# bluenote-1577/skani

Measured on NVIDIA H100. Metric: genome-pairs/sec, skani triangle 5k x 5 Mbp synthetic, higher is better.
Workload: dtype u64

## Files before the change

### skani_b200/csrc/seeding.cu

```cuda
#include <cub/cub.cuh>
#include <thrust/iterator/transform_iterator.h>

#include <algorithm>
#include <cstdlib>
#include <cstring>

#include "sk_core.cuh"
#include "sk_internal.h"

namespace sk {

uint64_t count_launch(sk_ctx* ctx, uint64_t n) {
  ctx->launches += n;
  return ctx->launches;
}

constexpr int PACK_THREADS = 256;
constexpr uint32_t UCOARSE_SHIFT = 8;

__device__ __forceinline__ uint32_t find_contig(const uint32_t* __restrict__ cuoff, uint32_t u, uint32_t lo_hint, uint32_t hi_hint) {
  uint32_t lo = lo_hint, hi = hi_hint;
  while (hi - lo > 1) {
    uint32_t mid = (lo + hi) >> 1;
    if (cuoff[mid] <= u) lo = mid; else hi = mid;
  }
  return lo;
}
__device__ __forceinline__ uint32_t contig_of_unit(const uint32_t* __restrict__ ucoarse, const uint32_t* __restrict__ cuoff, uint32_t u) {
  const uint32_t lo = __ldg(ucoarse + (u >> UCOARSE_SHIFT)), hi = __ldg(ucoarse + (u >> UCOARSE_SHIFT) + 1) + 1;
  return find_contig(cuoff, u, lo, hi);
}

__global__ void __launch_bounds__(PACK_THREADS)
pack_kernel(const uint8_t* __restrict__ ascii, const uint64_t* __restrict__ coff, const uint32_t* __restrict__ cuoff,
            const uint32_t* __restrict__ clen, const uint32_t* __restrict__ ucoarse, uint32_t u_begin, uint32_t n_units,
            uint64_t* __restrict__ P, uint32_t* __restrict__ NM, int small_n) {
  const uint32_t u = u_begin + blockIdx.x * PACK_THREADS + threadIdx.x;
  if (u >= n_units) return;
  const uint32_t ci = contig_of_unit(ucoarse, cuoff, u);
  const uint32_t ul = u - cuoff[ci];
  const uint32_t len = clen[ci];
  const uint32_t nvalid = min(32u, len - 32u * ul);
  const uint8_t* src = ascii + coff[ci] + 32ull * ul;
  const uintptr_t addr = (uintptr_t)src;
  const uint32_t* wp = (const uint32_t*)(addr & ~(uintptr_t)3);
  const uint32_t sh = (uint32_t)(addr & 3) * 8;
  const uint32_t nwords = (nvalid + (uint32_t)(addr & 3) + 3) >> 2;
  uint32_t w[9];
#pragma unroll
  for (int i = 0; i < 9; i++) w[i] = (i < (int)nwords) ? __ldg(wp + i) : 0u;
  uint64_t packed = 0;
  uint32_t nm = 0;
#pragma unroll
  for (int i = 0; i < 8; i++) {
    const uint32_t r = __funnelshift_r(w[i], w[i + 1], sh);
    uint32_t c8, n4;
    pack_word(r, c8, n4, small_n != 0);
    packed |= (uint64_t)c8 << (8 * i);
    nm |= n4 << (4 * i);
  }
  if (nvalid < 32u) { packed &= (1ull << (2 * nvalid)) - 1ull; nm &= (1u << nvalid) - 1u; }
  P[u] = packed;
  NM[u] = nm;
}

constexpr int HASH_THREADS = 128;

template <int V>
__device__ __forceinline__ uint64_t xorshift_var(uint64_t key, uint32_t s, uint32_t c) {
  const uint32_t lo = (uint32_t)key, hi = (uint32_t)(key >> 32);
  uint32_t hs, ls;
  asm("mul.hi.u32 %0, %1, %2;" : "=r"(hs) : "r"(hi), "r"(c));
  if (V == 1) ls = __funnelshift_r(lo, hi, s);
  else { uint32_t t; asm("mul.hi.u32 %0, %1, %2;" : "=r"(t) : "r"(lo), "r"(c)); ls = t + hi * c; }
  return ((uint64_t)(hi ^ hs) << 32) | (uint64_t)(lo ^ ls);
}
template <int V>
__device__ __forceinline__ uint32_t unit_pass_mask_var(uint64_t lo, uint64_t hi, uint32_t nm_lo, uint32_t nm_hi, uint32_t n, uint32_t ul,
                                                       uint32_t seed_mask32, uint64_t threshold, uint32_t c24, uint32_t c14, uint32_t c28) {
  const uint32_t valid = unit_valid_mask(n, ul);
  if (valid == 0) return 0;
  const uint64_t clo = ~lo, chi = ~hi;
  const uint64_t tlo = pair_reverse64(hi), thi = pair_reverse64(lo);
  const uint32_t c[4] = {(uint32_t)clo, (uint32_t)(clo >> 32), (uint32_t)chi, (uint32_t)(chi >> 32)};
  const uint32_t t[4] = {(uint32_t)tlo, (uint32_t)(tlo >> 32), (uint32_t)thi, (uint32_t)(thi >> 32)};
  uint32_t pass = 0;
#pragma unroll
  for (uint32_t j = 0; j < 32; j++) {
    const uint32_t orv = 24 + 2 * j, ofw = 62 - 2 * j;
    const uint32_t rs = funnel_r32(c[orv >> 5], c[(orv >> 5) + 1], orv & 31) & seed_mask32;
    const uint32_t fs = funnel_r32(t[ofw >> 5], t[(ofw >> 5) + 1], ofw & 31) & seed_mask32;
    const uint32_t seed = fs < rs ? fs : rs;
    uint64_t key = ~((uint64_t)seed * 0x200001ull);
    key = xorshift_var<V>(key, 24, c24);
    key = key * 265ull;
    key = xorshift_var<V>(key, 14, c14);
    key = key * 21ull;
    key = xorshift_var<V>(key, 28, c28);
    key = key * 0x80000001ull;
    if (key < threshold) pass |= 1u << j;
  }
  pass &= valid;
  if ((nm_lo | nm_hi) != 0 && pass != 0) pass &= ~unit_n_suppress_mask(n, ul, nm_lo, nm_hi, pass);
  return pass;
}

template <int V>
__global__ void __launch_bounds__(HASH_THREADS)
hashpass_kernel(const uint64_t* __restrict__ P, const uint32_t* __restrict__ NM, const uint32_t* __restrict__ ucoarse,
                const uint32_t* __restrict__ cuoff, const uint32_t* __restrict__ clen, uint32_t n_units,
                uint64_t seed_mask, uint64_t threshold, uint32_t* __restrict__ PM, uint32_t c24, uint32_t c14, uint32_t c28,
                uint32_t scalar_k) {
  uint32_t u = blockIdx.x * HASH_THREADS + threadIdx.x;
  if (u >= n_units) return;
  const uint64_t hi = P[u];
  const uint64_t lo_raw = u ? P[u - 1] : 0ull;
  const uint32_t nhi = NM[u];
  const uint32_t nlo_raw = u ? NM[u - 1] : 0u;
  const uint32_t ci = contig_of_unit(ucoarse, cuoff, u);
  const uint32_t ul = u - cuoff[ci];
  const uint32_t n = clen[ci];
  const uint64_t lo = ul ? lo_raw : 0ull;
  const uint32_t nlo = ul ? nlo_raw : 0u;
  if (V == 0) PM[u] = unit_pass_mask_fast(lo, hi, nlo, nhi, n, ul, (uint32_t)seed_mask, threshold, scalar_k);
  else PM[u] = unit_pass_mask_var<V>(lo, hi, nlo, nhi, n, ul, (uint32_t)seed_mask, threshold, c24, c14, c28);
}

__global__ void __launch_bounds__(256)
expand_kernel(const uint64_t* __restrict__ P, const uint32_t* __restrict__ ucoarse, const uint32_t* __restrict__ cuoff,
              const uint32_t* __restrict__ clocal, uint32_t n_units, const uint32_t* __restrict__ PM,
              const uint32_t* __restrict__ uoff, uint64_t seed_mask, uint64_t threshold_marker,
              uint32_t* __restrict__ pv_kmer, uint32_t* __restrict__ pv_pos, uint32_t* __restrict__ pv_cc,
              uint64_t* __restrict__ mkv) {
  uint32_t u = blockIdx.x * 256 + threadIdx.x;
  if (u >= n_units) return;
  uint32_t pass = PM[u];
  if (pass == 0) return;
  uint32_t ci = contig_of_unit(ucoarse, cuoff, u);
  uint32_t ul = u - cuoff[ci];
  uint64_t hi = P[u];
  uint64_t lo = ul ? P[u - 1] : 0ull;
  WindowCtx w = make_window_ctx(lo, hi);
  uint32_t o = uoff[u];
  uint32_t cl = clocal[ci];
  while (pass) {
    uint32_t j = __ffs(pass) - 1;
    pass &= pass - 1;
    bool canon;
    uint32_t seed = window_seed(w, j, seed_mask, &canon);
    pv_kmer[o] = seed;
    pv_pos[o] = 32u * ul + j;
    pv_cc[o] = (cl << 1) | (canon ? 1u : 0u);
    mkv[o] = (mm_hash64(seed) < threshold_marker) ? window_marker(w, j) : ~0ull;
    o++;
  }
}

__global__ void gather_u32_kernel(const uint32_t* __restrict__ src, const uint32_t* __restrict__ idx, uint32_t n,
                                  uint32_t src_len, uint32_t total, uint32_t* __restrict__ dst) {
  uint32_t i = blockIdx.x * blockDim.x + threadIdx.x;
  if (i >= n) return;
  uint32_t k = idx[i];
  dst[i] = (k >= src_len) ? total : src[k];
}

__global__ void gather_u32_tail_kernel(const uint32_t* __restrict__ src, const uint32_t* __restrict__ idx, uint32_t n,
                                       uint32_t src_len, const uint32_t* __restrict__ tail, int tail_is_mask,
                                       uint32_t* __restrict__ dst) {
  uint32_t i = blockIdx.x * blockDim.x + threadIdx.x;
  if (i >= n) return;
  uint32_t k = idx[i];
  if (k >= src_len) { const uint32_t t = tail[src_len - 1]; dst[i] = src[src_len - 1] + (tail_is_mask ? (uint32_t)__popc(t) : t); }
  else dst[i] = src[k];
}

__global__ void marker_flag_kernel(const uint64_t* __restrict__ mkv, uint32_t n, uint32_t* __restrict__ flag) {
  uint32_t i = blockIdx.x * blockDim.x + threadIdx.x;
  if (i < n) flag[i] = (mkv[i] != ~0ull) ? 1u : 0u;
}
__global__ void marker_scatter_kernel(const uint64_t* __restrict__ mkv, const uint32_t* __restrict__ scan, uint32_t n,
                                      uint64_t* __restrict__ out) {
  uint32_t i = blockIdx.x * blockDim.x + threadIdx.x;
  if (i < n && mkv[i] != ~0ull) out[scan[i]] = mkv[i];
}

__global__ void iota_local_kernel(const uint64_t* __restrict__ seg_off, uint32_t* __restrict__ vals) {
  uint32_t g = blockIdx.x;
  uint64_t b = seg_off[g], e = seg_off[g + 1];
  for (uint64_t i = b + (uint64_t)blockIdx.y * blockDim.x + threadIdx.x; i < e; i += (uint64_t)blockDim.x * gridDim.y) vals[i] = (uint32_t)(i - b);
}

__global__ void kview_keys_kernel(const uint64_t* __restrict__ seg_off, const uint32_t* __restrict__ pv_kmer, uint32_t kbits,
                                  uint32_t ibits, uint64_t* __restrict__ keys, uint32_t* __restrict__ vals) {
  const uint32_t g = blockIdx.x;
  const uint64_t b = seg_off[g], e = seg_off[g + 1];
  for (uint64_t i = b + (uint64_t)blockIdx.y * blockDim.x + threadIdx.x; i < e; i += (uint64_t)blockDim.x * gridDim.y) {
    const uint64_t k = ((uint64_t)g << kbits) | pv_kmer[i];
    if (ibits) keys[i] = (k << ibits) | (uint64_t)(i - b);
    else { keys[i] = k; vals[i] = (uint32_t)(i - b); }
  }
}
__global__ void marker_keys_kernel(const uint64_t* __restrict__ seg_off, uint64_t* __restrict__ mk) {
  const uint32_t g = blockIdx.x;
  const uint64_t b = seg_off[g], e = seg_off[g + 1];
  for (uint64_t i = b + (uint64_t)blockIdx.y * blockDim.x + threadIdx.x; i < e; i += (uint64_t)blockDim.x * gridDim.y) mk[i] |= (uint64_t)g << (2 * MARKER_K);
}


__global__ void kview_gather_kernel(const uint64_t* __restrict__ seg_off, const uint64_t* __restrict__ skmer,
                                    const uint32_t* __restrict__ perm, const uint32_t* __restrict__ pv_pos,
                                    const uint32_t* __restrict__ pv_cc, uint32_t* __restrict__ kv_pos,
                                    uint32_t* __restrict__ kv_cc, uint32_t* __restrict__ head, uint32_t ibits, uint32_t gshift,
                                    uint32_t n) {
  const uint32_t i = blockIdx.x * blockDim.x + threadIdx.x;
  if (i >= n) return;
  const uint64_t imask = (1ull << ibits) - 1;
  const uint64_t k = skmer[i];
  const uint64_t b = seg_off[k >> gshift];
  const uint32_t r = ibits ? (uint32_t)(k & imask) : perm[i];
  kv_pos[i] = pv_pos[b + r];
  kv_cc[i] = pv_cc[b + r];
  head[i] = (i == 0 || (k >> ibits) != (skmer[i - 1] >> ibits)) ? 1u : 0u;
}

__global__ void groups_kernel(const uint64_t* __restrict__ seg_off, const uint64_t* __restrict__ skmer, uint64_t kmask,
                              const uint32_t* __restrict__ head, const uint32_t* __restrict__ hscan,
                              uint32_t n_genomes, uint32_t* __restrict__ ukmer, uint32_t* __restrict__ ustart, uint32_t ibits,
                              uint32_t gshift, uint32_t n) {
  const uint32_t i = blockIdx.x * blockDim.x + threadIdx.x;
  if (i < n && head[i]) {
    const uint64_t k = skmer[i];
    const uint32_t g = (uint32_t)(k >> gshift);
    const uint32_t gid = hscan[i];
    ukmer[gid] = (uint32_t)((k >> ibits) & kmask);
    ustart[gid + g] = (uint32_t)(i - seg_off[g]);
  }
  if (i < n_genomes) {
    const uint32_t g = i;
    const uint64_t b = seg_off[g], e = seg_off[g + 1];
    const uint32_t next_gid = (e < n) ? hscan[e] : hscan[n - 1] + head[n - 1];
    ustart[next_gid + g] = (uint32_t)(e - b);
  }
}

__global__ void mult_kernel(const uint64_t* __restrict__ seg_off, const uint32_t* __restrict__ head,
                            const uint32_t* __restrict__ hscan, const uint32_t* __restrict__ perm,
                            const uint32_t* __restrict__ ustart, uint16_t* __restrict__ pv_mult,
                            const uint64_t* __restrict__ skmer, uint32_t ibits, uint32_t gshift, uint32_t n) {
  const uint32_t i = blockIdx.x * blockDim.x + threadIdx.x;
  if (i >= n) return;
  const uint64_t imask = (1ull << ibits) - 1;
  const uint64_t k = skmer[i];
  const uint32_t g = (uint32_t)(k >> gshift);
  const uint32_t gid = hscan[i] + head[i] - 1;
  const uint32_t cntv = ustart[gid + g + 1] - ustart[gid + g];
  const uint32_t r = ibits ? (uint32_t)(k & imask) : perm[i];
  pv_mult[seg_off[g] + r] = (uint16_t)min(cntv, 65535u);
}

__global__ void bucket_kernel(const uint64_t* __restrict__ uk_off, const uint32_t* __restrict__ ukmer, uint32_t shift,
                              uint32_t* __restrict__ ubucket) {
  const uint32_t g = blockIdx.x;
  const uint32_t* uk = ukmer + uk_off[g];
  const uint32_t n = (uint32_t)(uk_off[g + 1] - uk_off[g]);
  for (uint32_t b = threadIdx.x; b <= UBUCKETS; b += blockDim.x) {
    uint32_t lo = 0, hi = n;
    while (lo < hi) {
      uint32_t mid = (lo + hi) >> 1;
      if ((uk[mid] >> shift) < b) lo = mid + 1; else hi = mid;
    }
    ubucket[(size_t)g * (UBUCKETS + 1) + b] = lo;
  }
}

__global__ void marker_head_kernel(const uint64_t* __restrict__ seg_off, const uint64_t* __restrict__ mk,
                                   uint32_t* __restrict__ head) {
  uint32_t g = blockIdx.x;
  uint64_t b = seg_off[g], e = seg_off[g + 1];
  for (uint64_t i = b + (uint64_t)blockIdx.y * blockDim.x + threadIdx.x; i < e; i += (uint64_t)blockDim.x * gridDim.y) head[i] = (i == b || mk[i] != mk[i - 1]) ? 1u : 0u;
}
__global__ void marker_compact_kernel(const uint64_t* __restrict__ mk, const uint32_t* __restrict__ head,
                                      const uint32_t* __restrict__ hscan, uint32_t n, uint64_t mask, uint64_t* __restrict__ out) {
  uint32_t i = blockIdx.x * blockDim.x + threadIdx.x;
  if (i < n && head[i]) out[hscan[i]] = mk[i] & mask;
}
__global__ void gather_scan_at_kernel(const uint32_t* __restrict__ scan, const uint64_t* __restrict__ at, uint32_t n,
                                      uint64_t len, uint32_t total, uint64_t* __restrict__ out) {
  uint32_t i = blockIdx.x * blockDim.x + threadIdx.x;
  if (i < n) out[i] = (at[i] >= len) ? (uint64_t)total : (uint64_t)scan[at[i]];
}

__global__ void gather_scan_at_tail_kernel(const uint32_t* __restrict__ scan, const uint64_t* __restrict__ at, uint32_t n,
                                           uint64_t len, const uint32_t* __restrict__ flag, uint64_t* __restrict__ out) {
  uint32_t i = blockIdx.x * blockDim.x + threadIdx.x;
  if (i < n) out[i] = (at[i] >= len) ? (uint64_t)(scan[len - 1] + flag[len - 1]) : (uint64_t)scan[at[i]];
}

static void* mbox_alloc(sk_ctx* ctx, size_t bytes) {
  bytes = (bytes + 63) & ~(size_t)63;
  for (;;) {
    if (ctx->mbox_block < ctx->mbox_blocks.size()) {
      auto& b = ctx->mbox_blocks[ctx->mbox_block];
      if (ctx->mbox_pos + bytes <= b.second) { void* p = b.first + ctx->mbox_pos; ctx->mbox_pos += bytes; return p; }
      ctx->mbox_block++; ctx->mbox_pos = 0;
      continue;
    }
    uint8_t* p = nullptr;
// ... 156 lines not shown
    DTmp<uint32_t> vals, perm, head, hscan;
    DTmp<uint64_t> keys, skmer;
    SK_CUDA(keys.alloc(S, ctx)); SK_CUDA(skmer.alloc(S, ctx));
    SK_CUDA(head.alloc(S + 1, ctx)); SK_CUDA(hscan.alloc(S + 1, ctx));
    const uint32_t kbits = std::min(32u, 2 * set->sp.k);
    const uint32_t gbits = G > 1 ? 32 - (uint32_t)__builtin_clz(G - 1) : 0;
    const uint64_t kmask = (kbits >= 64) ? ~0ull : ((1ull << kbits) - 1);
    uint64_t max_rec = 1;
    for (uint32_t g = 0; g < G; g++) max_rec = std::max<uint64_t>(max_rec, set->seed_off[g + 1] - set->seed_off[g]);
    uint32_t ibits = max_rec > 1 ? 64 - (uint32_t)__builtin_clzll(max_rec - 1) : 1;
    if (ibits + kbits + gbits > 64 || getenv("SK_KVIEW_SORT_PAIRS")) ibits = 0;
    if (!ibits) { SK_CUDA(vals.alloc(S, ctx)); SK_CUDA(perm.alloc(S, ctx)); }
    kview_keys_kernel<<<dim3(G, 8), 256, 0, st>>>(d_seed_off.p, set->pv_kmer, kbits, ibits, keys.p, vals.p); count_launch(ctx);
    size_t tb = 0;
    DTmp<uint8_t> tmp;
    if (ibits) {
      SK_CUDA(cub::DeviceRadixSort::SortKeys(nullptr, tb, keys.p, skmer.p, (int)S, (int)ibits, (int)(ibits + kbits + gbits), st));
      SK_CUDA(tmp.alloc(tb, ctx));
      SK_CUDA(cub::DeviceRadixSort::SortKeys(tmp.p, tb, keys.p, skmer.p, (int)S, (int)ibits, (int)(ibits + kbits + gbits), st));
    } else {
      SK_CUDA(cub::DeviceRadixSort::SortPairs(nullptr, tb, keys.p, skmer.p, vals.p, perm.p, (int)S, 0, (int)(kbits + gbits), st));
      SK_CUDA(tmp.alloc(tb, ctx));
      SK_CUDA(cub::DeviceRadixSort::SortPairs(tmp.p, tb, keys.p, skmer.p, vals.p, perm.p, (int)S, 0, (int)(kbits + gbits), st));
    }
    count_launch(ctx);
    const uint32_t gshift = ibits + kbits;
    kview_gather_kernel<<<div_up(S, 256), 256, 0, st>>>(d_seed_off.p, skmer.p, perm.p, set->pv_pos, set->pv_cc, set->kv_pos,
                                                        set->kv_cc, head.p, ibits, gshift, (uint32_t)S); count_launch(ctx);
    SK_TRY(scan_exclusive<uint32_t>(ctx, head.p, hscan.p, S));
    DTmp<uint64_t> d_ukoff;
    SK_CUDA(d_ukoff.alloc(G + 1, ctx));
    gather_scan_at_tail_kernel<<<div_up(G + 1, 256), 256, 0, st>>>(hscan.p, d_seed_off.p, G + 1, S, head.p, d_ukoff.p); count_launch(ctx);
    SK_CUDA(cudaMemcpyAsync(h_ukoff, d_ukoff.p, (size_t)(G + 1) * 8, cudaMemcpyDeviceToHost, st));
    SK_CUDA(ctx->arena.alloc((void**)&set->ukmer, S * 4));
    SK_CUDA(ctx->arena.alloc((void**)&set->ustart, (size_t)(S + G + 1) * 4));
    groups_kernel<<<div_up(std::max<uint64_t>(S, G), 256), 256, 0, st>>>(d_seed_off.p, skmer.p, kmask, head.p, hscan.p, G, set->ukmer,
                                                                         set->ustart, ibits, gshift, (uint32_t)S); count_launch(ctx);
    mult_kernel<<<div_up(S, 256), 256, 0, st>>>(d_seed_off.p, head.p, hscan.p, perm.p, set->ustart, set->pv_mult, skmer.p, ibits, gshift,
                                                (uint32_t)S); count_launch(ctx);
  } else {
    set->U = 0;
    SK_CUDA(ctx->arena.alloc((void**)&set->ukmer, 4));
    SK_CUDA(ctx->arena.alloc((void**)&set->ustart, (size_t)(G + 1) * 4));
    SK_CUDA(cudaMemsetAsync(set->ustart, 0, (size_t)(G + 1) * 4, st));
    for (uint32_t g = 0; g <= G; g++) h_ukoff[g] = 0;
  }
  SK_CUDA(cudaStreamSynchronize(st));
  for (uint32_t g = 0; g <= G; g++) set->uk_off[g] = h_ukoff[g];
  set->U = (size_t)set->uk_off[G];
  const size_t MR = raw_mk_off[G];
  set->mk_off.assign(G + 1, 0);
  if (MR > 0) {
    if (MR >= (1ull << 31)) { ctx->err = "sub-batch has >= 2^31 markers"; return SK_ERR_PARAM; }
    SK_CUDA(d_rawmk_off.alloc(G + 1, ctx));
    SK_CUDA(h2d_small(ctx, d_rawmk_off.p, raw_mk_off, (G + 1) * 8));
    DTmp<uint64_t> sorted;
    SK_CUDA(sorted.alloc(MR, ctx));
    size_t tb = 0;
    const uint32_t mgbits = G > 1 ? 32 - (uint32_t)__builtin_clz(G - 1) : 0;
    const bool global_sort = 2 * MARKER_K + mgbits <= 64;
    DTmp<uint8_t> tmp;
    if (global_sort) {
      marker_keys_kernel<<<dim3(G, 8), 256, 0, st>>>(d_rawmk_off.p, d_marker_raw); count_launch(ctx);
      SK_CUDA(cub::DeviceRadixSort::SortKeys(nullptr, tb, d_marker_raw, sorted.p, (int)MR, 0, (int)(2 * MARKER_K + mgbits), st));
      SK_CUDA(tmp.alloc(tb, ctx));
      SK_CUDA(cub::DeviceRadixSort::SortKeys(tmp.p, tb, d_marker_raw, sorted.p, (int)MR, 0, (int)(2 * MARKER_K + mgbits), st));
    } else {
      SK_CUDA(cub::DeviceSegmentedRadixSort::SortKeys(nullptr, tb, d_marker_raw, sorted.p, (int)MR, (int)G, d_rawmk_off.p,
                                                      d_rawmk_off.p + 1, 0, 2 * MARKER_K, st));
      SK_CUDA(tmp.alloc(tb, ctx));
      SK_CUDA(cub::DeviceSegmentedRadixSort::SortKeys(tmp.p, tb, d_marker_raw, sorted.p, (int)MR, (int)G, d_rawmk_off.p,
                                                      d_rawmk_off.p + 1, 0, 2 * MARKER_K, st));
    }
    count_launch(ctx);
    DTmp<uint32_t> head, hscan;
    SK_CUDA(head.alloc(MR, ctx)); SK_CUDA(hscan.alloc(MR, ctx));
    marker_head_kernel<<<dim3(G, 8), 256, 0, st>>>(d_rawmk_off.p, sorted.p, head.p); count_launch(ctx);
    SK_TRY(scan_exclusive<uint32_t>(ctx, head.p, hscan.p, MR));
    SK_CUDA(ctx->arena.alloc((void**)&set->markers, MR * 8));
    marker_compact_kernel<<<div_up(MR, 256), 256, 0, st>>>(sorted.p, head.p, hscan.p, (uint32_t)MR, global_sort ? ((1ull << (2 * MARKER_K)) - 1) : ~0ull, set->markers); count_launch(ctx);
    DTmp<uint64_t> d_mkoff;
    SK_CUDA(d_mkoff.alloc(G + 1, ctx));
    gather_scan_at_tail_kernel<<<div_up(G + 1, 256), 256, 0, st>>>(hscan.p, d_rawmk_off.p, G + 1, MR, head.p, d_mkoff.p); count_launch(ctx);
    SK_CUDA(cudaMemcpyAsync(h_mkoff, d_mkoff.p, (size_t)(G + 1) * 8, cudaMemcpyDeviceToHost, st));
    SK_CUDA(cudaStreamSynchronize(st));
    for (uint32_t g = 0; g <= G; g++) set->mk_off[g] = h_mkoff[g];
    set->M = (size_t)set->mk_off[G];
  } else {
    set->M = 0;
    SK_CUDA(ctx->arena.alloc((void**)&set->markers, 8));
  }
  return SK_OK;
}

struct PopcOp { using result_type = uint32_t; __device__ __forceinline__ uint32_t operator()(uint32_t m) const { return (uint32_t)__popc(m); } };

int sketch_batch_device(sk_ctx* ctx, const SeedSrc& src, const uint64_t* contig_off, uint32_t n_contigs,
                        const uint32_t* genome_of_contig, uint32_t n_genomes, const sk_sketch_params* sp, sk_sketch_set** out) {
  cudaStream_t st = ctx->stream;
  const uint32_t G = n_genomes;
  sk_sketch_set* set = new sk_sketch_set();
  set->ctx = ctx; set->sp = *sp; set->G = G;
  struct Guard { sk_sketch_set* s; ~Guard() { if (s) { free_set_device(s); delete s; } } } guard{set};

  std::vector<uint64_t> coff(n_contigs + 1);
  std::vector<uint32_t> cuoff(n_contigs + 1), clen(n_contigs), clocal(n_contigs);
  set->ctg_off.assign(G + 1, 0);
  set->total_len.assign(G, 0);
  set->ctg_len.resize(n_contigs);
  uint64_t units = 0;
  uint32_t prev_g = 0, rank = 0;
  for (uint32_t i = 0; i < n_contigs; i++) {
    uint64_t len = contig_off[i + 1] - contig_off[i];
    if (contig_off[i + 1] < contig_off[i] || len >= (1ull << 32) - 65536) { ctx->err = "contig length out of range (u32 positions, src/types.rs:52; pos + 20000 must not wrap, src/chain.rs:743)"; return SK_ERR_PARAM; }
    uint32_t g = genome_of_contig[i];
    if (g >= G || g < prev_g) { ctx->err = "genome_of_contig must be non-decreasing and < n_genomes"; return SK_ERR_PARAM; }
    if (g != prev_g || i == 0) rank = 0;
    prev_g = g;
    if (rank >= (1u << 30)) { ctx->err = "contig index exceeds 30 bits (src/types.rs:136)"; return SK_ERR_PARAM; }
    coff[i] = contig_off[i] - src.ascii_base;
    cuoff[i] = (uint32_t)units;
    clen[i] = (uint32_t)len;
    clocal[i] = rank++;
    set->ctg_len[i] = (uint32_t)len;
    set->ctg_off[g + 1]++;
    set->total_len[g] += len;
    units += (len + 31) / 32;
    if (units >= (1ull << 31)) { ctx->err = "sub-batch too large (>= 2^31 units)"; return SK_ERR_PARAM; }
  }
  coff[n_contigs] = contig_off[n_contigs] - src.ascii_base;
  cuoff[n_contigs] = (uint32_t)units;
  for (uint32_t g = 0; g < G; g++) set->ctg_off[g + 1] += set->ctg_off[g];
  set->C = n_contigs;
  set->name_rank.resize(G);
  for (uint32_t g = 0; g < G; g++) set->name_rank[g] = g;
  const uint32_t NU = (uint32_t)units;
  const uint32_t n_packed = std::min(src.n_packed, n_contigs);
  if (n_packed && (!src.d_P || !src.d_NM)) { ctx->err = "packed contigs without unit arrays"; return SK_ERR_PARAM; }
  std::vector<uint32_t> ucoarse(((size_t)NU >> UCOARSE_SHIFT) + 2, n_contigs ? n_contigs - 1 : 0);
  {
    uint32_t ci = 0;
    for (size_t j = 0; ((uint64_t)j << UCOARSE_SHIFT) < NU; j++) {
      const uint32_t u = (uint32_t)(j << UCOARSE_SHIFT);
      while (ci + 1 < n_contigs && cuoff[ci + 1] <= u) ci++;
      ucoarse[j] = ci;
    }
  }

  SK_CUDA(ctx->arena.alloc((void**)&set->d_ctg_len, std::max<size_t>(n_contigs, 1) * 4));
  SK_CUDA(ctx->arena.alloc((void**)&set->ctg_rec_off, (size_t)(n_contigs + G + 1) * 4));
  set->seed_off.assign(G + 1, 0);

  DTmp<uint64_t> d_coff, Pown;
  DTmp<uint32_t> d_cuoff, d_clen, d_clocal, d_ucoarse, NMown, PM, uoff;
  mbox_reset(ctx);
  uint64_t* h_raw_mk_off = (uint64_t*)mbox_alloc(ctx, (size_t)(G + 1) * 8);
  if (h_raw_mk_off) for (uint32_t g = 0; g <= G; g++) h_raw_mk_off[g] = 0;
  DTmp<uint64_t> mkv, mraw;
  if (NU > 0) {
    SK_CUDA(d_coff.alloc(n_contigs + 1, ctx)); SK_CUDA(d_cuoff.alloc(n_contigs + 1, ctx));
    SK_CUDA(d_clen.alloc(n_contigs, ctx)); SK_CUDA(d_clocal.alloc(n_contigs, ctx)); SK_CUDA(d_ucoarse.alloc(ucoarse.size(), ctx));
    SK_CUDA(h2d_small(ctx, d_coff.p, coff.data(), (n_contigs + 1) * 8));
    SK_CUDA(h2d_small(ctx, d_cuoff.p, cuoff.data(), (n_contigs + 1) * 4));
    SK_CUDA(h2d_small(ctx, d_clen.p, clen.data(), n_contigs * 4));
    SK_CUDA(h2d_small(ctx, d_clocal.p, clocal.data(), n_contigs * 4));
    SK_CUDA(h2d_small(ctx, d_ucoarse.p, ucoarse.data(), ucoarse.size() * 4));
    SK_CUDA(h2d_small(ctx, set->d_ctg_len, clen.data(), n_contigs * 4));
    uint64_t* P = src.d_P; uint32_t* NM = src.d_NM;
    if (!P) { SK_CUDA(Pown.alloc(NU, ctx)); SK_CUDA(NMown.alloc(NU, ctx)); P = Pown.p; NM = NMown.p; }
    SK_CUDA(PM.alloc(NU, ctx)); SK_CUDA(uoff.alloc(NU, ctx));

    const uint32_t u_ascii = cuoff[n_packed];
    if (u_ascii < NU) {
      if (!src.d_ascii) { ctx->err = "ASCII contigs without a device buffer"; return SK_ERR_PARAM; }
      SK_LAUNCH(ctx, "pack_kernel", (pack_kernel<<<div_up(NU - u_ascii, PACK_THREADS), PACK_THREADS, 0, st>>>(
          src.d_ascii, d_coff.p, d_cuoff.p, d_clen.p, d_ucoarse.p, u_ascii, NU, P, NM, ctx->seed_scalar ? 1 : 0)));
    }
    const uint64_t seed_mask = ~0ull >> (64 - 2 * sp->k);
    const uint64_t thr = ~0ull / sp->c, thr_m = ~0ull / sp->marker_c;
    {
      const uint32_t scalar_k = ctx->seed_scalar ? sp->k : 0;
      const int hv = (getenv("SK_HASHPASS_VARIANT") && !scalar_k) ? atoi(getenv("SK_HASHPASS_VARIANT")) : 0;
      const uint32_t c24 = 1u << 8, c14 = 1u << 18, c28 = 1u << 4;
      const uint32_t grid = div_up(NU, HASH_THREADS);
      if (hv == 1) SK_LAUNCH(ctx, "hashpass_kernel", (hashpass_kernel<1><<<grid, HASH_THREADS, 0, st>>>(P, NM, d_ucoarse.p, d_cuoff.p, d_clen.p, NU, seed_mask, thr, PM.p, c24, c14, c28, scalar_k)));
      else if (hv == 2) SK_LAUNCH(ctx, "hashpass_kernel", (hashpass_kernel<2><<<grid, HASH_THREADS, 0, st>>>(P, NM, d_ucoarse.p, d_cuoff.p, d_clen.p, NU, seed_mask, thr, PM.p, c24, c14, c28, scalar_k)));
      else SK_LAUNCH(ctx, "hashpass_kernel", (hashpass_kernel<0><<<grid, HASH_THREADS, 0, st>>>(P, NM, d_ucoarse.p, d_cuoff.p, d_clen.p, NU, seed_mask, thr, PM.p, c24, c14, c28, scalar_k)));
    }
    {
      auto cnt_it = thrust::make_transform_iterator((const uint32_t*)PM.p, PopcOp());
      size_t tb = 0;
      SK_CUDA(cub::DeviceScan::ExclusiveSum(nullptr, tb, cnt_it, uoff.p, (int)NU, st));
      DTmp<uint8_t> tmp;
      SK_CUDA(tmp.alloc(tb, ctx));
      SK_CUDA(cub::DeviceScan::ExclusiveSum(tmp.p, tb, cnt_it, uoff.p, (int)NU, st));
      count_launch(ctx, 2);
    }
    DTmp<uint32_t> d_crec;
    SK_CUDA(d_crec.alloc(n_contigs + 1, ctx));
    gather_u32_tail_kernel<<<div_up(n_contigs + 1, 256), 256, 0, st>>>(uoff.p, d_cuoff.p, n_contigs + 1, NU, PM.p, 1, d_crec.p); count_launch(ctx);
    uint32_t* crec = (uint32_t*)mbox_alloc(ctx, (size_t)(n_contigs + 1) * 4);
    if (!crec || !h_raw_mk_off) { ctx->err = "out of pinned host memory"; return SK_ERR_NOMEM; }
    SK_CUDA(cudaMemcpyAsync(crec, d_crec.p, (size_t)(n_contigs + 1) * 4, cudaMemcpyDeviceToHost, st));
    SK_CUDA(cudaStreamSynchronize(st));
    const uint32_t S = crec[n_contigs];
    set->S = S;
    SK_CUDA(ctx->arena.alloc((void**)&set->pv_kmer, std::max<size_t>(S, 1) * 4));
    SK_CUDA(ctx->arena.alloc((void**)&set->pv_pos, std::max<size_t>(S, 1) * 4));
    SK_CUDA(ctx->arena.alloc((void**)&set->pv_cc, std::max<size_t>(S, 1) * 4));
    SK_CUDA(mkv.alloc(S, ctx));
    SK_LAUNCH(ctx, "expand_kernel", (expand_kernel<<<div_up(NU, 256), 256, 0, st>>>(
        P, d_ucoarse.p, d_cuoff.p, d_clocal.p, NU, PM.p, uoff.p, seed_mask, thr_m, set->pv_kmer, set->pv_pos, set->pv_cc, mkv.p)));
    std::vector<uint32_t> crl(n_contigs + G + 1, 0);
    for (uint32_t g = 0; g < G; g++) {
      uint64_t c0 = set->ctg_off[g], c1 = set->ctg_off[g + 1];
      uint32_t base = (c0 < n_contigs) ? crec[c0] : S;
      set->seed_off[g] = base;
      for (uint64_t c = c0; c < c1; c++) crl[c + g] = crec[c] - base;
      uint32_t endrec = (c1 < n_contigs) ? crec[c1] : S;
      crl[c1 + g] = endrec - base;
    }
    set->seed_off[G] = S;
    SK_CUDA(h2d_small(ctx, set->ctg_rec_off, crl.data(), (size_t)(n_contigs + G) * 4));
    if (S > 0) {
      DTmp<uint32_t> mflag, mscan;
      SK_CUDA(mflag.alloc(S, ctx)); SK_CUDA(mscan.alloc(S, ctx));
      marker_flag_kernel<<<div_up(S, 256), 256, 0, st>>>(mkv.p, S, mflag.p); count_launch(ctx);
      SK_TRY(scan_exclusive<uint32_t>(ctx, mflag.p, mscan.p, S));
      DTmp<uint64_t> d_so, d_mo;
      SK_CUDA(d_so.alloc(G + 1, ctx)); SK_CUDA(d_mo.alloc(G + 1, ctx));
      SK_CUDA(h2d_small(ctx, d_so.p, set->seed_off.data(), (G + 1) * 8));
      SK_CUDA(mraw.alloc(S, ctx));
      marker_scatter_kernel<<<div_up(S, 256), 256, 0, st>>>(mkv.p, mscan.p, S, mraw.p); count_launch(ctx);
      gather_scan_at_tail_kernel<<<div_up(G + 1, 256), 256, 0, st>>>(mscan.p, d_so.p, G + 1, S, mflag.p, d_mo.p); count_launch(ctx);
      SK_CUDA(cudaMemcpyAsync(h_raw_mk_off, d_mo.p, (size_t)(G + 1) * 8, cudaMemcpyDeviceToHost, st));
    }
  } else {
    set->S = 0;
    SK_CUDA(ctx->arena.alloc((void**)&set->pv_kmer, 4)); SK_CUDA(ctx->arena.alloc((void**)&set->pv_pos, 4)); SK_CUDA(ctx->arena.alloc((void**)&set->pv_cc, 4));
    SK_CUDA(cudaMemsetAsync(set->ctg_rec_off, 0, (size_t)(n_contigs + G + 1) * 4, st));
  }
  Pown.release(); NMown.release(); PM.release(); uoff.release(); mkv.release();
  if (!h_raw_mk_off) { ctx->err = "out of pinned host memory"; return SK_ERR_NOMEM; }
  SK_TRY(build_views(ctx, set, mraw.p, h_raw_mk_off));
  SK_CUDA(cudaStreamSynchronize(st));
  guard.s = nullptr;
  *out = set;
  return SK_OK;
}

}
```

### skani_b200/csrc/sk_core.cuh

```cuda
#pragma once
#include <stdint.h>

#if defined(__CUDACC__)
#define SK_HD __host__ __device__ __forceinline__
#else
#define SK_HD inline
#endif

namespace sk {

constexpr int MARKER_K = 21;
constexpr uint32_t UNIT_BASES = 32;

SK_HD uint64_t mm_hash64(uint64_t key) {
  key = ~(key + (key << 21));
  key = key ^ (key >> 24);
  key = key * 265;
  key = key ^ (key >> 14);
  key = key * 21;
  key = key ^ (key >> 28);
  key = key + (key << 31);
  return key;
}

// ... 56 lines not shown
  w.t_lo = pair_reverse64(hi); w.t_hi = pair_reverse64(lo);
  return w;
}
SK_HD uint64_t window_f21(const WindowCtx& w, uint32_t j) { return extract128(w.t_lo, w.t_hi, 62 - 2 * j) & ((1ull << 42) - 1); }
SK_HD uint64_t window_r21(const WindowCtx& w, uint32_t j) { return extract128(w.c_lo, w.c_hi, 24 + 2 * j) & ((1ull << 42) - 1); }

SK_HD uint32_t window_seed(const WindowCtx& w, uint32_t j, uint64_t seed_mask, bool* canonical) {
  uint64_t fs = window_f21(w, j) & seed_mask;
  uint64_t rs = window_r21(w, j) & seed_mask;
  *canonical = fs < rs;
  return (uint32_t)(fs < rs ? fs : rs);
}
SK_HD uint64_t window_marker(const WindowCtx& w, uint32_t j) {
  uint64_t f = window_f21(w, j), r = window_r21(w, j);
  return r > f ? f : r;
}

SK_HD uint32_t unit_valid_mask(uint32_t n, uint32_t ul) {
  if (n < 2 * MARKER_K) return 0;
  uint32_t q = (n - 20) / 4;
  uint64_t e_lo = 20, e_hi = 4ull * q + 20;
  uint64_t b = 32ull * ul;
  uint32_t m = 0xFFFFFFFFu;
  if (b + 32 <= e_lo || b >= e_hi) return 0;
  if (b < e_lo) m &= 0xFFFFFFFFu << (uint32_t)(e_lo - b);
  if (b + 32 > e_hi) m &= 0xFFFFFFFFu >> (uint32_t)(b + 32 - e_hi);
  return m;
}

SK_HD uint32_t unit_n_suppress_mask(uint32_t n, uint32_t ul, uint32_t nm_lo, uint32_t nm_hi, uint32_t cand) {
  uint64_t nm = ((uint64_t)nm_hi << 32) | nm_lo;
  if (nm == 0 || cand == 0) return 0;
  uint32_t q = (n - 20) / 4;
  uint32_t sup = 0;
  for (uint32_t j = 0; j < 32; j++) {
    if (!((cand >> j) & 1u)) continue;
    int64_t e = 32ll * ul + j;
    int64_t lane = (e - 20) / (int64_t)q;
    int64_t lb = e - 20;
    int64_t lane_lb = lane * (int64_t)q + 20;
    if (lane_lb > lb) lb = lane_lb;
    int64_t base0 = 32ll * ((int64_t)ul - 1);
    uint32_t r_lo = (uint32_t)(lb - base0), r_hi = (uint32_t)(e - base0);
    uint64_t span = (r_hi - r_lo == 63) ? ~0ull : (((1ull << (r_hi - r_lo + 1)) - 1) << r_lo);
    if (nm & span) sup |= 1u << j;
  }
  return sup;
}

SK_HD uint32_t unit_valid_mask_scalar(uint32_t n, uint32_t ul) {
  if (n < 2 * MARKER_K) return 0;
  const uint64_t e_lo = 20, e_hi = n;
  const uint64_t b = 32ull * ul;
  uint32_t m = 0xFFFFFFFFu;
  if (b + 32 <= e_lo || b >= e_hi) return 0;
  if (b < e_lo) m &= 0xFFFFFFFFu << (uint32_t)(e_lo - b);
  if (b + 32 > e_hi) m &= 0xFFFFFFFFu >> (uint32_t)(b + 32 - e_hi);
  return m;
}
SK_HD uint32_t unit_n_suppress_mask_scalar(uint32_t ul, uint32_t k, uint32_t nm_lo, uint32_t nm_hi, uint32_t cand) {
  const uint64_t nm = ((uint64_t)nm_hi << 32) | nm_lo;
  if (nm == 0 || cand == 0) return 0;
  uint32_t sup = 0;
  for (uint32_t j = 0; j < 32; j++) {
    if (!((cand >> j) & 1u)) continue;
    const int64_t e = 32ll * ul + j;
    int64_t lb = e - (int64_t)k + 1;
    if (lb < 20) lb = 20;
    const int64_t base0 = 32ll * ((int64_t)ul - 1);
    const uint32_t r_lo = (uint32_t)(lb - base0), r_hi = (uint32_t)(e - base0);
    const uint64_t span = (((r_hi - r_lo == 63) ? ~0ull : ((1ull << (r_hi - r_lo + 1)) - 1)) << r_lo);
    if (nm & span) sup |= 1u << j;
  }
  return sup;
}

}

namespace sk {

SK_HD uint32_t unit_pass_mask(uint64_t lo, uint64_t hi, uint32_t nm_lo, uint32_t nm_hi, uint32_t n, uint32_t ul,
                              uint64_t seed_mask, uint64_t threshold) {
  uint32_t valid = unit_valid_mask(n, ul);
  if (valid == 0) return 0;
  WindowCtx w = make_window_ctx(lo, hi);
  uint32_t pass = 0;
#if defined(__CUDA_ARCH__)
#pragma unroll
#endif
  for (uint32_t j = 0; j < 32; j++) {
    uint64_t fs = window_f21(w, j) & seed_mask;
    uint64_t rs = window_r21(w, j) & seed_mask;
    uint64_t seed = fs < rs ? fs : rs;
    if (mm_hash64(seed) < threshold) pass |= 1u << j;
  }
  pass &= valid;
  if ((nm_lo | nm_hi) != 0 && pass != 0) pass &= ~unit_n_suppress_mask(n, ul, nm_lo, nm_hi, pass);
  return pass;
}

}

namespace sk {

SK_HD uint32_t funnel_r32(uint32_t lo, uint32_t hi, uint32_t sh) {
#if defined(__CUDA_ARCH__)
  return __funnelshift_r(lo, hi, sh);
#else
  return sh ? (lo >> sh) | (hi << (32 - sh)) : lo;
#endif
}
SK_HD uint64_t mm_hash64_mul(uint64_t key) {
  {
    const uint64_t k = key * 0x200001ull;
    const uint32_t a = (uint32_t)k, b = (uint32_t)(k >> 32);
    const uint32_t lo = a ^ funnel_r32(a, b, 24);
    const uint32_t hi = b ^ (b >> 24) ^ 0xFFFFFF00u;
    key = ((uint64_t)hi << 32) | lo;
  }
  key = key * 265ull;
  key = key ^ (key >> 14);
  key = key * 21ull;
  key = key ^ (key >> 28);
  key = key * 0x80000001ull;
  return key;
}

SK_HD uint32_t unit_pass_mask_fast(uint64_t lo, uint64_t hi, uint32_t nm_lo, uint32_t nm_hi, uint32_t n, uint32_t ul,
                                   uint32_t seed_mask32, uint64_t threshold, uint32_t scalar_k = 0) {
  const uint32_t valid = scalar_k ? unit_valid_mask_scalar(n, ul) : unit_valid_mask(n, ul);
  if (valid == 0) return 0;
  const uint64_t clo = ~lo, chi = ~hi;
  const uint64_t tlo = pair_reverse64(hi), thi = pair_reverse64(lo);
  const uint32_t c[4] = {(uint32_t)clo, (uint32_t)(clo >> 32), (uint32_t)chi, (uint32_t)(chi >> 32)};
  const uint32_t t[4] = {(uint32_t)tlo, (uint32_t)(tlo >> 32), (uint32_t)thi, (uint32_t)(thi >> 32)};
  uint32_t pass = 0;
#if defined(__CUDA_ARCH__)
#pragma unroll
#endif
  for (uint32_t j = 0; j < 32; j++) {
    const uint32_t orv = 24 + 2 * j;
    const uint32_t ofw = 62 - 2 * j;
    const uint32_t rs = funnel_r32(c[orv >> 5], c[(orv >> 5) + 1], orv & 31) & seed_mask32;
    const uint32_t fs = funnel_r32(t[ofw >> 5], t[(ofw >> 5) + 1], ofw & 31) & seed_mask32;
    const uint32_t seed = fs < rs ? fs : rs;
    if (mm_hash64_mul((uint64_t)seed) < threshold) pass |= 1u << j;
  }
  pass &= valid;
  if ((nm_lo | nm_hi) != 0 && pass != 0)
    pass &= ~(scalar_k ? unit_n_suppress_mask_scalar(ul, scalar_k, nm_lo, nm_hi, pass) : unit_n_suppress_mask(n, ul, nm_lo, nm_hi, pass));
  return pass;
}

}

namespace sk {

enum ScreenMode { MODE_QUICK = 0, MODE_QUICK_NORESCUE = 1, MODE_INDEX = 2, MODE_INDEX_NORESCUE = 3, MODE_TRIANGLE = 4 };
constexpr uint64_t SCREEN_MINIMUM_KMERS = 20;

SK_HD bool screen_row_rescued(int mode, bool rescue_small, uint64_t card_row) {
  return (mode == MODE_TRIANGLE || mode == MODE_INDEX) && rescue_small && card_row < SCREEN_MINIMUM_KMERS;
}

SK_HD bool screen_pass(int mode, bool rescue_small, uint64_t card_row, uint64_t card_col, uint64_t count, double cutoff) {
  const uint64_t mn = card_row < card_col ? card_row : card_col;
  if (mode == MODE_TRIANGLE || mode == MODE_INDEX || mode == MODE_INDEX_NORESCUE) {
    if (screen_row_rescued(mode, rescue_small, card_row)) return true;
    unsigned long long thr = (unsigned long long)(cutoff * (double)mn);
    if (thr < 1) thr = 1;
    return count > thr;
  }
  const bool rescue = (mode == MODE_QUICK) && rescue_small;
  if (mn < SCREEN_MINIMUM_KMERS && rescue) return true;
  if (mn == 0) return rescue;
  unsigned long long ratio = (unsigned long long)(cutoff * (double)mn);
  if (ratio == 0) ratio = 1;
  return count >= ratio;
}

}
```

Measured before the change: 47.31 million.

## Fuse ASCII packing into hashpass, add fast ACGT pack path, block-balance expand

Replaces the separate pack kernel with a hashpass_ascii kernel that packs ASCII units, exchanges the previous unit's packed word through warp shuffles (lane 0 repacks its predecessor cooperatively), and computes pass masks in one launch. This drops the NM array and one global round trip. A fast path uses byte_perm to pack words that hold only uppercase ACGT. The expand kernel now gives each block 1024 units, block-scans the popcounts and spreads the emitted seeds evenly across threads, at the cost of a binary search per output. These stages are seeding work, and seeding is probably a small part of all-pairs triangle throughput.

```diff
diff --git a/skani_b200/csrc/seeding.cu b/skani_b200/csrc/seeding.cu
--- a/skani_b200/csrc/seeding.cu
+++ b/skani_b200/csrc/seeding.cu
@@ -15,7 +15,6 @@
   return ctx->launches;
 }
 
-constexpr int PACK_THREADS = 256;
 constexpr uint32_t UCOARSE_SHIFT = 8;
 
 __device__ __forceinline__ uint32_t find_contig(const uint32_t* __restrict__ cuoff, uint32_t u, uint32_t lo_hint, uint32_t hi_hint) {
@@ -29,39 +28,6 @@
 __device__ __forceinline__ uint32_t contig_of_unit(const uint32_t* __restrict__ ucoarse, const uint32_t* __restrict__ cuoff, uint32_t u) {
   const uint32_t lo = __ldg(ucoarse + (u >> UCOARSE_SHIFT)), hi = __ldg(ucoarse + (u >> UCOARSE_SHIFT) + 1) + 1;
   return find_contig(cuoff, u, lo, hi);
-}
-
-__global__ void __launch_bounds__(PACK_THREADS)
-pack_kernel(const uint8_t* __restrict__ ascii, const uint64_t* __restrict__ coff, const uint32_t* __restrict__ cuoff,
-            const uint32_t* __restrict__ clen, const uint32_t* __restrict__ ucoarse, uint32_t u_begin, uint32_t n_units,
-            uint64_t* __restrict__ P, uint32_t* __restrict__ NM, int small_n) {
-  const uint32_t u = u_begin + blockIdx.x * PACK_THREADS + threadIdx.x;
-  if (u >= n_units) return;
-  const uint32_t ci = contig_of_unit(ucoarse, cuoff, u);
-  const uint32_t ul = u - cuoff[ci];
-  const uint32_t len = clen[ci];
-  const uint32_t nvalid = min(32u, len - 32u * ul);
-  const uint8_t* src = ascii + coff[ci] + 32ull * ul;
-  const uintptr_t addr = (uintptr_t)src;
-  const uint32_t* wp = (const uint32_t*)(addr & ~(uintptr_t)3);
-  const uint32_t sh = (uint32_t)(addr & 3) * 8;
-  const uint32_t nwords = (nvalid + (uint32_t)(addr & 3) + 3) >> 2;
-  uint32_t w[9];
-#pragma unroll
-  for (int i = 0; i < 9; i++) w[i] = (i < (int)nwords) ? __ldg(wp + i) : 0u;
-  uint64_t packed = 0;
-  uint32_t nm = 0;
-#pragma unroll
-  for (int i = 0; i < 8; i++) {
-    const uint32_t r = __funnelshift_r(w[i], w[i + 1], sh);
-    uint32_t c8, n4;
-    pack_word(r, c8, n4, small_n != 0);
-    packed |= (uint64_t)c8 << (8 * i);
-    nm |= n4 << (4 * i);
-  }
-  if (nvalid < 32u) { packed &= (1ull << (2 * nvalid)) - 1ull; nm &= (1u << nvalid) - 1u; }
-  P[u] = packed;
-  NM[u] = nm;
 }
 
 constexpr int HASH_THREADS = 128;
@@ -106,6 +72,14 @@
 }
 
 template <int V>
+__device__ __forceinline__ uint32_t unit_pass(uint64_t lo, uint64_t hi, uint32_t nlo, uint32_t nhi, uint32_t n, uint32_t ul,
+                                              uint32_t seed_mask32, uint64_t threshold, uint32_t c24, uint32_t c14, uint32_t c28,
+                                              uint32_t scalar_k) {
+  if (V == 0) return unit_pass_mask_fast(lo, hi, nlo, nhi, n, ul, seed_mask32, threshold, scalar_k);
+  return unit_pass_mask_var<V>(lo, hi, nlo, nhi, n, ul, seed_mask32, threshold, c24, c14, c28);
+}
+
+template <int V>
 __global__ void __launch_bounds__(HASH_THREADS)
 hashpass_kernel(const uint64_t* __restrict__ P, const uint32_t* __restrict__ NM, const uint32_t* __restrict__ ucoarse,
                 const uint32_t* __restrict__ cuoff, const uint32_t* __restrict__ clen, uint32_t n_units,
@@ -122,37 +96,97 @@
   const uint32_t n = clen[ci];
   const uint64_t lo = ul ? lo_raw : 0ull;
   const uint32_t nlo = ul ? nlo_raw : 0u;
-  if (V == 0) PM[u] = unit_pass_mask_fast(lo, hi, nlo, nhi, n, ul, (uint32_t)seed_mask, threshold, scalar_k);
-  else PM[u] = unit_pass_mask_var<V>(lo, hi, nlo, nhi, n, ul, (uint32_t)seed_mask, threshold, c24, c14, c28);
-}
-
-__global__ void __launch_bounds__(256)
+  PM[u] = unit_pass<V>(lo, hi, nlo, nhi, n, ul, (uint32_t)seed_mask, threshold, c24, c14, c28, scalar_k);
+}
+
+template <int V>
+__global__ void __launch_bounds__(HASH_THREADS)
+hashpass_ascii_kernel(const uint8_t* __restrict__ ascii, const uint64_t* __restrict__ coff, const uint32_t* __restrict__ ucoarse,
+                      const uint32_t* __restrict__ cuoff, const uint32_t* __restrict__ clen, uint32_t u_begin, uint32_t n_units,
+                      uint64_t seed_mask, uint64_t threshold, uint64_t* __restrict__ P, uint32_t* __restrict__ PM,
+                      uint32_t c24, uint32_t c14, uint32_t c28, uint32_t scalar_k) {
+  const uint32_t u = u_begin + blockIdx.x * HASH_THREADS + threadIdx.x;
+  const uint32_t lane = threadIdx.x & 31u;
+  const bool live = u < n_units;
+  const bool small_n = scalar_k != 0;
+  uint32_t ul = 0, n = 0, nhi = 0;
+  uint64_t hi = 0;
+  const uint8_t* src = ascii;
+  if (live) {
+    const uint32_t ci = contig_of_unit(ucoarse, cuoff, u);
+    ul = u - cuoff[ci];
+    n = clen[ci];
+    src = ascii + coff[ci] + 32ull * ul;
+    pack_unit_ascii(src, min(32u, n - 32u * ul), small_n, hi, nhi);
+  }
+  uint64_t lo = __shfl_up_sync(0xFFFFFFFFu, hi, 1);
+  uint32_t nlo = __shfl_up_sync(0xFFFFFFFFu, nhi, 1);
+  if (__shfl_sync(0xFFFFFFFFu, ul, 0) != 0) {
+    const uint8_t* prev = (const uint8_t*)__shfl_sync(0xFFFFFFFFu, (unsigned long long)src, 0) - 32;
+    uint32_t c8 = 0, n4 = 0;
+    if (lane < 8) pack_word_ascii(prev + 4 * lane, small_n, c8, n4);
+    const uint32_t plo = __reduce_or_sync(0xFFFFFFFFu, lane < 4 ? c8 << (8 * lane) : 0u);
+    const uint32_t phi = __reduce_or_sync(0xFFFFFFFFu, lane >= 4 ? c8 << (8 * (lane & 3)) : 0u);
+    const uint32_t pn = __reduce_or_sync(0xFFFFFFFFu, n4 << (4 * (lane & 7)));
+    if (lane == 0) { lo = ((uint64_t)phi << 32) | plo; nlo = pn; }
+  }
+  if (!live) return;
+  if (ul == 0) { lo = 0; nlo = 0; }
+  P[u] = hi;
+  PM[u] = unit_pass<V>(lo, hi, nlo, nhi, n, ul, (uint32_t)seed_mask, threshold, c24, c14, c28, scalar_k);
+}
+
+constexpr int EXPAND_THREADS = 256, EXPAND_UPT = 4, EXPAND_UNITS = EXPAND_THREADS * EXPAND_UPT;
+__global__ void __launch_bounds__(EXPAND_THREADS)
 expand_kernel(const uint64_t* __restrict__ P, const uint32_t* __restrict__ ucoarse, const uint32_t* __restrict__ cuoff,
               const uint32_t* __restrict__ clocal, uint32_t n_units, const uint32_t* __restrict__ PM,
               const uint32_t* __restrict__ uoff, uint64_t seed_mask, uint64_t threshold_marker,
               uint32_t* __restrict__ pv_kmer, uint32_t* __restrict__ pv_pos, uint32_t* __restrict__ pv_cc,
               uint64_t* __restrict__ mkv) {
-  uint32_t u = blockIdx.x * 256 + threadIdx.x;
-  if (u >= n_units) return;
-  uint32_t pass = PM[u];
-  if (pass == 0) return;
-  uint32_t ci = contig_of_unit(ucoarse, cuoff, u);
-  uint32_t ul = u - cuoff[ci];
-  uint64_t hi = P[u];
-  uint64_t lo = ul ? P[u - 1] : 0ull;
-  WindowCtx w = make_window_ctx(lo, hi);
-  uint32_t o = uoff[u];
-  uint32_t cl = clocal[ci];
-  while (pass) {
-    uint32_t j = __ffs(pass) - 1;
-    pass &= pass - 1;
+  using Scan = cub::BlockScan<uint32_t, EXPAND_THREADS>;
+  __shared__ typename Scan::TempStorage scan_tmp;
+  __shared__ uint32_t s_off[EXPAND_UNITS], s_pm[EXPAND_UNITS];
+  const uint32_t u0 = blockIdx.x * EXPAND_UNITS;
+  const uint32_t t = threadIdx.x;
+  uint32_t pm[EXPAND_UPT], cnt[EXPAND_UPT];
+  if (u0 + EXPAND_UNITS <= n_units) {
+    const uint4 v = *reinterpret_cast<const uint4*>(PM + u0 + EXPAND_UPT * t);
+    pm[0] = v.x; pm[1] = v.y; pm[2] = v.z; pm[3] = v.w;
+  } else {
+#pragma unroll
+    for (int k = 0; k < EXPAND_UPT; k++) pm[k] = (u0 + EXPAND_UPT * t + k < n_units) ? PM[u0 + EXPAND_UPT * t + k] : 0u;
+  }
+#pragma unroll
+  for (int k = 0; k < EXPAND_UPT; k++) cnt[k] = (uint32_t)__popc(pm[k]);
+  uint32_t total;
+  Scan(scan_tmp).ExclusiveSum(cnt, cnt, total);
+#pragma unroll
+  for (int k = 0; k < EXPAND_UPT; k++) { s_off[EXPAND_UPT * t + k] = cnt[k]; s_pm[EXPAND_UPT * t + k] = pm[k]; }
+  __syncthreads();
+  if (total == 0) return;
+  const uint32_t base = uoff[u0];
+  for (uint32_t r = t; r < total; r += EXPAND_THREADS) {
+    uint32_t lo_i = 0, hi_i = EXPAND_UNITS;
+    while (hi_i - lo_i > 1) {
+      const uint32_t mid = (lo_i + hi_i) >> 1;
+      if (s_off[mid] <= r) lo_i = mid; else hi_i = mid;
+    }
+    uint32_t pass = s_pm[lo_i];
+    for (uint32_t k = r - s_off[lo_i]; k; k--) pass &= pass - 1;
+    const uint32_t j = __ffs(pass) - 1;
+    const uint32_t u = u0 + lo_i;
+    const uint32_t ci = contig_of_unit(ucoarse, cuoff, u);
+    const uint32_t ul = u - cuoff[ci];
+    const uint64_t hi = P[u];
+    const uint64_t lo = ul ? P[u - 1] : 0ull;
+    const WindowCtx w = make_window_ctx(lo, hi);
+    const uint32_t o = base + r;
     bool canon;
-    uint32_t seed = window_seed(w, j, seed_mask, &canon);
+    const uint32_t seed = window_seed(w, j, seed_mask, &canon);
     pv_kmer[o] = seed;
     pv_pos[o] = 32u * ul + j;
-    pv_cc[o] = (cl << 1) | (canon ? 1u : 0u);
+    pv_cc[o] = (clocal[ci] << 1) | (canon ? 1u : 0u);
     mkv[o] = (mm_hash64(seed) < threshold_marker) ? window_marker(w, j) : ~0ull;
-    o++;
   }
 }
 
@@ -615,7 +649,7 @@
   set->seed_off.assign(G + 1, 0);
 
   DTmp<uint64_t> d_coff, Pown;
-  DTmp<uint32_t> d_cuoff, d_clen, d_clocal, d_ucoarse, NMown, PM, uoff;
+  DTmp<uint32_t> d_cuoff, d_clen, d_clocal, d_ucoarse, PM, uoff;
   mbox_reset(ctx);
   uint64_t* h_raw_mk_off = (uint64_t*)mbox_alloc(ctx, (size_t)(G + 1) * 8);
   if (h_raw_mk_off) for (uint32_t g = 0; g <= G; g++) h_raw_mk_off[g] = 0;
@@ -629,26 +663,32 @@
     SK_CUDA(h2d_small(ctx, d_clocal.p, clocal.data(), n_contigs * 4));
     SK_CUDA(h2d_small(ctx, d_ucoarse.p, ucoarse.data(), ucoarse.size() * 4));
     SK_CUDA(h2d_small(ctx, set->d_ctg_len, clen.data(), n_contigs * 4));
-    uint64_t* P = src.d_P; uint32_t* NM = src.d_NM;
-    if (!P) { SK_CUDA(Pown.alloc(NU, ctx)); SK_CUDA(NMown.alloc(NU, ctx)); P = Pown.p; NM = NMown.p; }
+    uint64_t* P = src.d_P;
+    if (!P) { SK_CUDA(Pown.alloc(NU, ctx)); P = Pown.p; }
     SK_CUDA(PM.alloc(NU, ctx)); SK_CUDA(uoff.alloc(NU, ctx));
 
     const uint32_t u_ascii = cuoff[n_packed];
-    if (u_ascii < NU) {
-      if (!src.d_ascii) { ctx->err = "ASCII contigs without a device buffer"; return SK_ERR_PARAM; }
-      SK_LAUNCH(ctx, "pack_kernel", (pack_kernel<<<div_up(NU - u_ascii, PACK_THREADS), PACK_THREADS, 0, st>>>(
-          src.d_ascii, d_coff.p, d_cuoff.p, d_clen.p, d_ucoarse.p, u_ascii, NU, P, NM, ctx->seed_scalar ? 1 : 0)));
-    }
+    if (u_ascii < NU && !src.d_ascii) { ctx->err = "ASCII contigs without a device buffer"; return SK_ERR_PARAM; }
     const uint64_t seed_mask = ~0ull >> (64 - 2 * sp->k);
     const uint64_t thr = ~0ull / sp->c, thr_m = ~0ull / sp->marker_c;
     {
       const uint32_t scalar_k = ctx->seed_scalar ? sp->k : 0;
       const int hv = (getenv("SK_HASHPASS_VARIANT") && !scalar_k) ? atoi(getenv("SK_HASHPASS_VARIANT")) : 0;
       const uint32_t c24 = 1u << 8, c14 = 1u << 18, c28 = 1u << 4;
-      const uint32_t grid = div_up(NU, HASH_THREADS);
-      if (hv == 1) SK_LAUNCH(ctx, "hashpass_kernel", (hashpass_kernel<1><<<grid, HASH_THREADS, 0, st>>>(P, NM, d_ucoarse.p, d_cuoff.p, d_clen.p, NU, seed_mask, thr, PM.p, c24, c14, c28, scalar_k)));
-      else if (hv == 2) SK_LAUNCH(ctx, "hashpass_kernel", (hashpass_kernel<2><<<grid, HASH_THREADS, 0, st>>>(P, NM, d_ucoarse.p, d_cuoff.p, d_clen.p, NU, seed_mask, thr, PM.p, c24, c14, c28, scalar_k)));
-      else SK_LAUNCH(ctx, "hashpass_kernel", (hashpass_kernel<0><<<grid, HASH_THREADS, 0, st>>>(P, NM, d_ucoarse.p, d_cuoff.p, d_clen.p, NU, seed_mask, thr, PM.p, c24, c14, c28, scalar_k)));
+      if (u_ascii > 0) {
+        const uint32_t grid = div_up(u_ascii, HASH_THREADS);
+        const uint32_t* NM = src.d_NM;
+        if (hv == 1) SK_LAUNCH(ctx, "hashpass_kernel", (hashpass_kernel<1><<<grid, HASH_THREADS, 0, st>>>(P, NM, d_ucoarse.p, d_cuoff.p, d_clen.p, u_ascii, seed_mask, thr, PM.p, c24, c14, c28, scalar_k)));
+        else if (hv == 2) SK_LAUNCH(ctx, "hashpass_kernel", (hashpass_kernel<2><<<grid, HASH_THREADS, 0, st>>>(P, NM, d_ucoarse.p, d_cuoff.p, d_clen.p, u_ascii, seed_mask, thr, PM.p, c24, c14, c28, scalar_k)));
+        else SK_LAUNCH(ctx, "hashpass_kernel", (hashpass_kernel<0><<<grid, HASH_THREADS, 0, st>>>(P, NM, d_ucoarse.p, d_cuoff.p, d_clen.p, u_ascii, seed_mask, thr, PM.p, c24, c14, c28, scalar_k)));
+      }
+      if (u_ascii < NU) {
+        const uint32_t grid = div_up(NU - u_ascii, HASH_THREADS);
+        const uint8_t* A = src.d_ascii;
+        if (hv == 1) SK_LAUNCH(ctx, "hashpass_kernel", (hashpass_ascii_kernel<1><<<grid, HASH_THREADS, 0, st>>>(A, d_coff.p, d_ucoarse.p, d_cuoff.p, d_clen.p, u_ascii, NU, seed_mask, thr, P, PM.p, c24, c14, c28, scalar_k)));
+        else if (hv == 2) SK_LAUNCH(ctx, "hashpass_kernel", (hashpass_ascii_kernel<2><<<grid, HASH_THREADS, 0, st>>>(A, d_coff.p, d_ucoarse.p, d_cuoff.p, d_clen.p, u_ascii, NU, seed_mask, thr, P, PM.p, c24, c14, c28, scalar_k)));
+        else SK_LAUNCH(ctx, "hashpass_kernel", (hashpass_ascii_kernel<0><<<grid, HASH_THREADS, 0, st>>>(A, d_coff.p, d_ucoarse.p, d_cuoff.p, d_clen.p, u_ascii, NU, seed_mask, thr, P, PM.p, c24, c14, c28, scalar_k)));
+      }
     }
     {
       auto cnt_it = thrust::make_transform_iterator((const uint32_t*)PM.p, PopcOp());
@@ -672,7 +712,7 @@
     SK_CUDA(ctx->arena.alloc((void**)&set->pv_pos, std::max<size_t>(S, 1) * 4));
     SK_CUDA(ctx->arena.alloc((void**)&set->pv_cc, std::max<size_t>(S, 1) * 4));
     SK_CUDA(mkv.alloc(S, ctx));
-    SK_LAUNCH(ctx, "expand_kernel", (expand_kernel<<<div_up(NU, 256), 256, 0, st>>>(
+    SK_LAUNCH(ctx, "expand_kernel", (expand_kernel<<<div_up(NU, EXPAND_UNITS), EXPAND_THREADS, 0, st>>>(
         P, d_ucoarse.p, d_cuoff.p, d_clocal.p, NU, PM.p, uoff.p, seed_mask, thr_m, set->pv_kmer, set->pv_pos, set->pv_cc, mkv.p)));
     std::vector<uint32_t> crl(n_contigs + G + 1, 0);
     for (uint32_t g = 0; g < G; g++) {
@@ -703,7 +743,7 @@
     SK_CUDA(ctx->arena.alloc((void**)&set->pv_kmer, 4)); SK_CUDA(ctx->arena.alloc((void**)&set->pv_pos, 4)); SK_CUDA(ctx->arena.alloc((void**)&set->pv_cc, 4));
     SK_CUDA(cudaMemsetAsync(set->ctg_rec_off, 0, (size_t)(n_contigs + G + 1) * 4, st));
   }
-  Pown.release(); NMown.release(); PM.release(); uoff.release(); mkv.release();
+  Pown.release(); PM.release(); uoff.release(); mkv.release();
   if (!h_raw_mk_off) { ctx->err = "out of pinned host memory"; return SK_ERR_NOMEM; }
   SK_TRY(build_views(ctx, set, mraw.p, h_raw_mk_off));
   SK_CUDA(cudaStreamSynchronize(st));
diff --git a/skani_b200/csrc/sk_core.cuh b/skani_b200/csrc/sk_core.cuh
--- a/skani_b200/csrc/sk_core.cuh
+++ b/skani_b200/csrc/sk_core.cuh
@@ -232,6 +232,77 @@
   return pass;
 }
 
+SK_HD uint32_t load_word32(const uint32_t* p) {
+#if defined(__CUDA_ARCH__)
+  return __ldg(p);
+#else
+  uint32_t v;
+  __builtin_memcpy(&v, p, 4);
+  return v;
+#endif
+}
+
+SK_HD uint32_t byte_perm(uint32_t a, uint32_t b, uint32_t s) {
+#if defined(__CUDA_ARCH__)
+  return __byte_perm(a, b, s);
+#else
+  const uint64_t v = ((uint64_t)b << 32) | a;
+  uint32_t r = 0;
+  for (int k = 0; k < 4; k++) r |= (uint32_t)((v >> (8 * ((s >> (4 * k)) & 7))) & 0xFFu) << (8 * k);
+  return r;
+#endif
+}
+
+SK_HD void pack_unit_ascii(const uint8_t* src, uint32_t nvalid, bool small_n, uint64_t& packed, uint32_t& nm) {
+  const uintptr_t addr = (uintptr_t)src;
+  const uint32_t* wp = (const uint32_t*)(addr & ~(uintptr_t)3);
+  const uint32_t sh = (uint32_t)(addr & 3) * 8;
+  const uint32_t nwords = (nvalid + (uint32_t)(addr & 3) + 3) >> 2;
+  uint32_t w[9];
+#if defined(__CUDA_ARCH__)
+#pragma unroll
+#endif
+  for (int i = 0; i < 9; i++) w[i] = (i < (int)nwords) ? load_word32(wp + i) : 0u;
+  uint32_t r[8], y[8], bad1 = 0, bad2 = 0;
+#if defined(__CUDA_ARCH__)
+#pragma unroll
+#endif
+  for (int i = 0; i < 8; i++) {
+    r[i] = funnel_r32(w[i], w[i + 1], sh);
+    const uint32_t s1 = r[i] >> 1, lh = s1 & ~r[i];
+    bad1 |= ((r[i] >> 3) ^ lh) | ~((r[i] << 1) | lh);
+    bad2 |= r[i] ^ 0x40404040u;
+    y[i] = ((s1 ^ r[i]) & 0x06060606u) * 0x00820820u;
+  }
+  if (((bad1 & 0x02020202u) | (bad2 & 0xC8C8C8C8u)) == 0u) {
+    const uint32_t lo = byte_perm(byte_perm(y[0], y[1], 0x0073u), byte_perm(y[2], y[3], 0x7300u), 0x7610u);
+    const uint32_t hi = byte_perm(byte_perm(y[4], y[5], 0x0073u), byte_perm(y[6], y[7], 0x7300u), 0x7610u);
+    packed = ((uint64_t)hi << 32) | lo;
+    nm = 0;
+  } else {
+    packed = 0;
+    nm = 0;
+#if defined(__CUDA_ARCH__)
+#pragma unroll
+#endif
+    for (int i = 0; i < 8; i++) {
+      uint32_t c8, n4;
+      pack_word(r[i], c8, n4, small_n);
+      packed |= (uint64_t)c8 << (8 * i);
+      nm |= n4 << (4 * i);
+    }
+  }
+  if (nvalid < 32u) { packed &= (1ull << (2 * nvalid)) - 1ull; nm &= (1u << nvalid) - 1u; }
+}
+
+SK_HD void pack_word_ascii(const uint8_t* src, bool small_n, uint32_t& c8, uint32_t& n4) {
+  const uintptr_t addr = (uintptr_t)src;
+  const uint32_t* wp = (const uint32_t*)(addr & ~(uintptr_t)3);
+  const uint32_t sh = (uint32_t)(addr & 3) * 8;
+  const uint32_t w0 = load_word32(wp), w1 = sh ? load_word32(wp + 1) : 0u;
+  pack_word(funnel_r32(w0, w1, sh), c8, n4, small_n);
+}
+
 }
 
 namespace sk {
```

Measured after the change: 50.19 million, median of 6. 6.1% higher.
